# peterdavidfagan/mujoco_robot_environments

Measured on AMD Instinct MI355X. Metric: env steps/sec (whole node), RearrangementEnv batch=4096 at 1/2/4/8 MI355X, higher is better.
Workload: dtype f32

## Files before the change

### mujoco_robot_environments_amd/csrc/mre_kernels.hip

```cpp
#include <hip/hip_runtime.h>

#include "mre_dev.h"
#include "mre_math.h"
#include "mre_collide.h"

namespace mre {
using ModelP = MRE_MODEL_PTR(DevModel);
#if defined(MRE_PHASE_STAMPS) && MRE_PHASE_STAMPS >= 4
__shared__ unsigned long long dbg_acc[4];
#endif

struct OscSm {
  float J[6][7], M[7][7], MiJt[7][6], Li[6][6], Lam[6][6], V[6][6], Jbar[7][6];
  float ep[3], eo[3], F[6], LF[6], tn[7], Jbt[6], xd[6], w[6];
};

struct alignas(8) Blk {
  uint16_t row0;
  uint8_t type, nrows;
  uint8_t rslot;
  uint8_t pa, pb;
  uint8_t primary : 4;
  uint8_t bslot : 4;
};
// ... 18 lines not shown
#endif
  float cdof[NRV][6];
  union {
    struct { float con_pos[NCON_MAX][3], con_frame[NCON_MAX][9], con_dist[NCON_MAX]; };
#ifdef MRE_NEWTON
    struct { float jar[NEFC_MAX], frc[NEFC_MAX], jv[NEFC_MAX]; };
#else
    struct { float jar[NEFC_MAX], frc[NEFC_MAX], pyr_f[4 * NCON_MAX]; };
#endif
  };
  float com_robot[3];
  float site_xpos[NSITE][3], site_xmat[1][9];
#ifdef MRE_NEWTON
  float qM[NMR];
#else
  float qM[NMR], qLD[NMR], qLDinv[NRV + 1];
#endif
  float prop_mass[NPROP], prop_inertia[NPROP][3], prop_size[NPROP][3];
  union { float scratch[64]; int iscr[64]; };
  float osc_tgt[16];
  int nprops;
  int ncon, nefc, nl, nrrow, npp, overflow, solver_iters;
  int finger_contact;
  uint8_t con_pair[NCON_MAX], con_rslot[NCON_MAX], con_bslot[NCON_MAX], con_b1[NCON_MAX], con_b2[NCON_MAX];
  uint16_t lim_info[NRV + 1];
  union {
    float JpA[3 * NCON_MAX][6];
    struct {
      float cinert[NB][10], crb[NRB][10], gP[NRB - GRIP_BODY0][6], gC[NRB - GRIP_BODY0][6];
      double gpose[NRB - GRIP_BODY0][7];
    };
  };
  float JpB[3 * NPP_MAX][6];
  union {
    float Jr[NRROW_MAX][NRV];
    struct {
      float cdof_dot[NV][6], cvel[NB][6], cfrc[NB][6];
      alignas(8) double gI[NRB - GRIP_BODY0][10];
      double gS[NRB - GRIP_BODY0][6];
    };
  };
#ifdef MRE_NEWTON
  float efc_R[NEFC_MAX], efc_aref[NEFC_MAX];
  float frc_r[NRROW_MAX];
  float con_fric[NCON_MAX];
  float hc[NCON_MAX][6];
  float Md[NRV][MD_LD];
  alignas(8) float W[NV * (NV + 1) / 2];
  uint8_t rstate[NEFC_MAX];
  uint8_t clist[NPROP][NCON_MAX];
  uint8_t ccount[NPROP], cpl_robot, cpl_cubes;
  alignas(8) uint16_t jdesc[NEFC_MAX][4];
  float zrow[24];
#else
  float Br[NRROW_MAX][NRV];
  alignas(16) float blkrec[MAXBLK][16];
  Blk blk[MAXBLK];
  uint8_t sched[MAXBLK][8];
#endif
  uint16_t hdr[NEFC_MAX];

  int nblk, nsched;
};

#if defined(MRE_LARGE_CAPS)
static_assert(sizeof(Sm) <= 27136, "large-capacity Sm must fit 6 workgroups per CU");
#else
static_assert(sizeof(Sm) <= 20480, "compact Sm must fit 8 workgroups per CU");
#endif

#ifdef MRE_NEWTON
MRE_DEV float* mh_store(Sm& s) { return &s.JpA[0][0]; }
static_assert(sizeof(((Sm*)0)->JpA) >= sizeof(float) * NMR, "M - h dF/dv fits the head of the constraint block");
#else
MRE_DEV float* mh_store(Sm& s) { return s.qLD; }
#endif

struct BodyRegs {
  float anchor[3], axis[3], xipos[3], ximat[9];
};

MRE_DEV double robot_q(const Sm& s, int d) { return (double)s.qpos[d] + (double)s.qlo[d]; }
MRE_DEV double robot_v(const Sm& s, int d) { return (double)s.qvel[d] + (double)s.qlo[QFINE / 2 + d]; }

MRE_DEV bool prop_is_active(const Sm& s, int propid) { return propid < 0 || propid < s.nprops; }

struct BodyK {
  float quat[4], pos[3], mass, jnt_pos[3], qpos0, jnt_axis[3], ipos[3], iquat[4], inertia[3];
  int qposadr, propid, dofadr, parent;
};
MRE_DEV BodyK load_body(ModelP M, int b) {
  const auto* R = &M->body_rec[b];
  BodyK B;
#pragma unroll
  for (int k = 0; k < 4; k++) { B.quat[k] = R->quat[k]; B.iquat[k] = R->iquat[k]; }
#pragma unroll
  for (int k = 0; k < 3; k++) { B.pos[k] = R->pos[k]; B.jnt_pos[k] = R->jnt_pos[k]; B.jnt_axis[k] = R->jnt_axis[k];
                                B.ipos[k] = R->ipos[k]; B.inertia[k] = R->inertia[k]; }
  B.mass = R->mass; B.qpos0 = R->qpos0; B.qposadr = R->qposadr; B.propid = R->propid; B.dofadr = R->dofadr;
  B.parent = R->parent;
  return B;
}

MRE_DEV bool body_is_active(ModelP M, const Sm& s, int b) {
  int p = M->body_propid[b];
  return p < 0 || p < s.nprops;
}

MRE_DEV void sincos_poly_d(double x, double& sn, double& cs) {
  const double z = x * x;
  double ps = -1.0 / 1307674368000.0;
  ps = ps * z + 1.0 / 6227020800.0;
  ps = ps * z - 1.0 / 39916800.0;
  ps = ps * z + 1.0 / 362880.0;
  ps = ps * z - 1.0 / 5040.0;
  ps = ps * z + 1.0 / 120.0;
  ps = ps * z - 1.0 / 6.0;
  sn = x + x * (z * ps);
  double pc = 1.0 / 20922789888000.0;
  pc = pc * z - 1.0 / 87178291200.0;
  pc = pc * z + 1.0 / 479001600.0;
// ... 1163 lines not shown
  ModelP M = (ModelP)a.M;

  const bool save = a.sv_qpos != nullptr && step_lo == 0;
  if (l < NQP) {
    const float v = a.qpos[(size_t)env * NQP + l];
    s.qpos[l] = v;
    if (save) a.sv_qpos[(size_t)env * NQP + l] = v;
  }
  if (l < NVP) {
    const float v = a.qvel[(size_t)env * NVP + l], w = a.qacc_ws[(size_t)env * NVP + l];
    s.qvel[l] = v;
    s.qacc[l] = w;
    s.qfrc_con[l] = 0.f;
    if (save) { a.sv_qvel[(size_t)env * NVP + l] = v; a.sv_qacc_ws[(size_t)env * NVP + l] = w; }
  }
  if (l < QFINE) {
    const float v = a.qfine != nullptr ? a.qfine[(size_t)env * QFINE_ROW + l] : 0.f;
    s.qlo[l] = v;
    if (save && a.qfine != nullptr) a.sv_qfine[(size_t)env * QFINE_ROW + l] = v;
  }
  if (save && a.qfine != nullptr && l < QFINE_ROW - QFINE)
    a.sv_qfine[(size_t)env * QFINE_ROW + QFINE + l] = a.qfine[(size_t)env * QFINE_ROW + QFINE + l];
  float cube_lo_keep = 0.f;
  if (QUEUE && !Q_LARGE && a.qfine != nullptr && l < QFINE_ROW - QFINE) cube_lo_keep = a.qfine[(size_t)env * QFINE_ROW + QFINE + l];
  if (l < NU) {
    const float v = a.ctrl[(size_t)env * NU + l];
    s.ctrl[l] = v;
    if (save) a.sv_ctrl[(size_t)env * NU + l] = v;
  }
  if (save && l == 0) {
    if (a.nstep != nullptr) a.sv_nstep[env] = a.nstep[env];
    a.sv_status[env] = a.status[env];
    a.sv_converged[env] = a.converged != nullptr ? a.converged[env] : (uint8_t)0;
  }
  if (l == 0) { s.nprops = a.nprops[env]; s.overflow = 0; s.ncon = 0; s.nefc = 0; s.solver_iters = 0; }
#ifdef MRE_NEWTON
  if (l < 24) s.zrow[l] = 0.f;
#endif
  if (l < NPROP * 3) {
    const float sz = a.prop_size[(size_t)env * NPROP * 3 + l];
    s.prop_size[l / 3][l % 3] = sz;
  }
  MRE_SYNC();
  if (l < NPROP) {
    const float m = M->body_mass[NRB + l];
    const float* z = s.prop_size[l];
    s.prop_mass[l] = m;
    s.prop_inertia[l][0] = m / 3.f * (z[1] * z[1] + z[2] * z[2]);
    s.prop_inertia[l][1] = m / 3.f * (z[0] * z[0] + z[2] * z[2]);
    s.prop_inertia[l][2] = m / 3.f * (z[0] * z[0] + z[1] * z[1]);
  }
  MRE_SYNC();

#if defined(MRE_PHASE_STAMPS) && MRE_PHASE_STAMPS >= 4
  if (l < 4) dbg_acc[l] = 0ull;
#endif
#ifdef MRE_PHASE_STAMPS
  unsigned long long stamp_acc[4] = {0, 0, 0, 0};
  unsigned long long stamp_t = __builtin_amdgcn_s_memtime();
#endif
  bool arm_converged = ((a.flags & F_CONV_CONTINUE) != 0 || (QUEUE && qtick > 0)) && a.converged != nullptr && a.converged[env] != 0;
  float grip_cmd = 0.f;
  const OscConfig* oscp = a.osc + (size_t)env * a.osc_stride;
  int hw_ncon = 0, hw_nefc = 0, hw_nrrow = 0, hw_npp = 0;
  const unsigned long long launch_t0 = __builtin_amdgcn_s_memtime();
  if (a.mode == CTRL_OSC) {
    if (l < 16) s.osc_tgt[l] = a.osc_target[(size_t)env * 16 + l];
    grip_cmd = a.grip_closed[env] ? M->act_ctrlrange[NU - 1][1] : M->act_ctrlrange[NU - 1][0];
    MRE_SYNC();
  }
  int steps_done = 0;
  bool settled = false;
  for (int step = step_lo; step < step_hi; ++step) {
    MRE_STAMP(7);
    position_stage(M, s, l);
    MRE_STAMP(12);
    MRE_STAMP(13);
    gripper_local(M, s, l);
    if ((a.flags & F_NO_CONSTRAINTS) == 0) connect_rows_local(M, s, l);
    MRE_STAMP(14);
    crb_mass_matrix(M, s, l);
    MRE_SYNC();
#ifndef MRE_NEWTON
    factor_robot_regs(s.qM, s.qLD, s.qLDinv);
#endif
    MRE_STAMP(15);
    MRE_STAMP(0);

    velocity_stage(M, s, l);
    MRE_SYNC();
    finger_bias(M, s, l);
    MRE_STAMP(1);
    const bool constrained = (a.flags & F_NO_CONSTRAINTS) == 0;
    if (constrained) {

      collide(M, s, l, false, (a.flags & F_CLIP_ALWAYS) != 0);
      MRE_STAMP(2);
      assemble_constraints(M, s, l);
#ifdef MRE_NEWTON
      nw_build_lists(s, l, a.flags);
#else
      solve_robot_rows(s, l);
      assemble_blocks(M, s, l);
#endif
      MRE_STAMP(3);
      hw_ncon = max(hw_ncon, s.ncon); hw_nefc = max(hw_nefc, s.nefc);
// ... 614 lines not shown
```

### mujoco_robot_environments_amd/csrc/mre_newton.h

```cpp
#pragma once

namespace mre {

constexpr int NW_QUAD = 0, NW_SAT = 1, NW_CONE = 4;
constexpr unsigned NW_CPL_ALL_TILES = 0x80u;
constexpr int NW_LS_MAX = 20;
constexpr float NW_LS_TOL = 0.01f;
#ifndef NW_LS_REL_VALUE
#define NW_LS_REL_VALUE 1e-5f
#endif
constexpr float NW_LS_REL = NW_LS_REL_VALUE;

MRE_DEV float rdlane(float v, int lane) {
  return __builtin_bit_cast(float, __builtin_amdgcn_readlane(__builtin_bit_cast(int, v), lane));
}
MRE_DEV int uni(int v) { return __builtin_amdgcn_readfirstlane(v); }
MRE_DEV float unif(float v) {
  return __builtin_bit_cast(float, __builtin_amdgcn_readfirstlane(__builtin_bit_cast(int, v)));
}

MRE_DEV float nw_Jl(const Sm& s, int i, int h, int l, int lp, int lk) {
  const int rs = h & 0xFF, pa = (h >> 8) & 0xF, pb = (h >> 12) & 0xF;
  float j = 0.f;
  if (l < NRV) {
// ... 71 lines not shown
  }
  return o;
}

template <bool FULL, bool PYR>
MRE_DEV float nw_update(Sm& s, int l, int nscalar, int ncon, float mu_scale, const float* jar) {
  constexpr bool pyr = PYR;
  float cost = 0.f;
  if (l < nscalar) {
    const float D = 1.0f / s.efc_R[l], j = jar[l];
    const bool act = l < 7 || j < 0.f;
    if (FULL) {
      const float f = act ? -D * j : 0.f;
      s.frc[l] = f; s.frc_r[l] = f;
      s.rstate[l] = act ? NW_QUAD : NW_SAT;
    }
    cost = act ? 0.5f * D * j * j : 0.f;
  }
  if (l < ncon) {
    const int i = nscalar + 3 * l;
    const float D0 = 1.0f / s.efc_R[i], D1 = 1.0f / s.efc_R[i + 1], D2 = 1.0f / s.efc_R[i + 2];
    const float fr = s.con_fric[l];
    float hc[6];
    const NwContact o = pyr ? nw_pyramid<FULL>(jar[i], jar[i + 1], jar[i + 2], D0, fr, hc)
                            : nw_contact<FULL>(jar[i], jar[i + 1], jar[i + 2], D0, D1, D2, fr, fr * mu_scale, hc);
    cost += o.cost;
    if (FULL) {
      s.frc[i] = o.f0; s.frc[i + 1] = o.f1; s.frc[i + 2] = o.f2;
      const int rs = s.con_rslot[l];
      if (rs != HDR_NONE) { s.frc_r[rs] = o.f0; s.frc_r[rs + 1] = o.f1; s.frc_r[rs + 2] = o.f2; }
      s.rstate[i] = s.rstate[i + 1] = s.rstate[i + 2] = (uint8_t)o.st;
      if (o.st == NW_CONE) {
#pragma unroll
        for (int k = 0; k < 6; k++) s.hc[l][k] = hc[k];
      }
    }
  }
  return wave_sum(cost);
}

struct NwMasks { unsigned long long sc, cq, cc; };
MRE_DEV bool operator==(const NwMasks& a, const NwMasks& b) { return a.sc == b.sc && a.cq == b.cq && a.cc == b.cc; }
MRE_DEV NwMasks nw_masks(const Sm& s, int l, int nscalar, int ncon) {
  NwMasks m;
  const int st_s = l < nscalar ? s.rstate[l] : NW_SAT;
  const int st_c = l < ncon ? s.rstate[nscalar + 3 * l] : NW_SAT;
  m.sc = __ballot(st_s == NW_QUAD);
  m.cq = __ballot(st_c == NW_QUAD);
  m.cc = __ballot(st_c == NW_CONE);
  return m;
}

MRE_DEV float nw_JTf(const Sm& s, int l, int lp, int lk, int nscalar) {
  float acc = 0.f;
  if (l < NRV) {
    const int n = s.nrrow;
    for (int rs = 0; rs < n; rs++) acc = fmaf(s.Jr[rs][l], s.frc_r[rs], acc);
  } else if (l < NV && lp < s.nprops) {
    const int n = s.ccount[lp];
    for (int t = 0; t < n; t++) {
      const int e = s.clist[lp][t], c = e & 0x7F;
      const float* J = (e & 0x80) ? s.JpB[3 * s.con_bslot[c]] : s.JpA[3 * c];
      const float* f = &s.frc[nscalar + 3 * c];
      acc = fmaf(J[lk], f[0], acc);
      acc = fmaf(J[6 + lk], f[1], acc);
      acc = fmaf(J[12 + lk], f[2], acc);
    }
  }
  return acc;
}

MRE_DEV void nw_rank1(float (&hh)[NV], float t, float J, bool has_r, int pa, int pb) {
  if (has_r) {
#pragma unroll
    for (int c = 0; c < NRV; c++) hh[c] = fmaf(t, rdlane(J, c), hh[c]);
  }
#pragma unroll
  for (int p = 0; p < NPROP; p++) {
    if (pa == p || pb == p) {
#pragma unroll
      for (int k = 0; k < 6; k++) hh[NRV + 6 * p + k] = fmaf(t, rdlane(J, NRV + 6 * p + k), hh[NRV + 6 * p + k]);
    }
  }
}

template <int HI, int LO>
MRE_DEV void nw_elim_update(float (&hh)[NV], float u) {
  constexpr int n = HI - LO + 1;
  if constexpr (n > 0) {
#pragma unroll
    for (int g0 = 0; g0 < n; g0 += 8) {
      float t[8];
#pragma unroll
      for (int q = 0; q < 8; q++)
        if (g0 + q < n) t[q] = rdlane(u, HI - g0 - q);
      __builtin_amdgcn_sched_barrier(0);
#pragma unroll
      for (int q = 0; q < 8; q++)
        if (g0 + q < n) hh[HI - g0 - q] = fmaf(-u, t[q], hh[HI - g0 - q]);
      __builtin_amdgcn_sched_barrier(0);
    }
  }
}

template <int K>
MRE_DEV void nw_elim_col(float (&hh)[NV], float& g, float& y, float& dinv, int l, unsigned nbm) {
// ... 11 lines not shown
  if constexpr (blk > 0) {
    if constexpr (blk > 3) { if (nbm & (1u << 3)) nw_elim_update<NRV + 17, NRV + 12>(hh, u); }
    if constexpr (blk > 2) { if (nbm & (1u << 2)) nw_elim_update<NRV + 11, NRV + 6>(hh, u); }
    if constexpr (blk > 1) { if (nbm & (1u << 1)) nw_elim_update<NRV + 5, NRV>(hh, u); }
    if (nbm & 1u) nw_elim_update<NRV - 1, 0>(hh, u);
  }
}
template <int K, int KEND>
MRE_DEV void nw_elim_range(float (&hh)[NV], float& g, float& y, float& dinv, int l, unsigned nbm) {
  nw_elim_col<K>(hh, g, y, dinv, l, nbm);
  if constexpr (K > KEND) nw_elim_range<K - 1, KEND>(hh, g, y, dinv, l, nbm);
}

struct NwPoint { float alpha, cost, d1, d2; };

MRE_PHASE_FN void nw_build_lists(Sm& s, int l, unsigned flags) {
  const int kept = s.ncon;
  const bool on = l < kept;
  const int cb1 = on ? s.con_b1[l] : 0, cb2 = on ? s.con_b2[l] : 0;
  int pa = -1, pb = -1;
  if (cb1 >= NRB) pa = cb1 - NRB;
  if (cb2 >= NRB) { if (pa < 0) pa = cb2 - NRB; else pb = cb2 - NRB; }
  const unsigned long long lt = (1ull << l) - 1ull;
  const bool rob = on && pa >= 0 && s.con_rslot[on ? l : 0] != HDR_NONE;
  unsigned cr = 0u, cc = 0u;
#pragma unroll
  for (int p = 0; p < NPROP; p++) {
    const bool mine = on && (pa == p || pb == p);
    const unsigned long long m = __ballot(mine);
    if (mine) s.clist[p][__popcll(m & lt)] = (uint8_t)(pb == p ? (l | 0x80) : l);
    if (l == 0) s.ccount[p] = (uint8_t)__popcll(m);
    if (__ballot(rob && pa == p) != 0ull) cr |= 1u << p;
  }
  const int pairbit = (on && pb >= 0) ? cube_pair_bit(pa, pb) : -1;
#pragma unroll
  for (int b = 0; b < 6; b++)
    if (__ballot(pairbit == b) != 0ull) cc |= 1u << b;
  if ((flags & F_NW_ALL_TILES) != 0u) cr |= NW_CPL_ALL_TILES;
  if (l == 0) { s.cpl_robot = (uint8_t)cr; s.cpl_cubes = (uint8_t)cc; }
  const int nscalar = 7 + s.nl;
  const unsigned zoff = (unsigned)offsetof(Sm, zrow);
  for (int i = l; i < s.nefc; i += 64) {
    const int h = s.hdr[i], ra = (h >> 8) & 0xF, rb = (h >> 12) & 0xF;
    const int crow = i - nscalar;
    const unsigned offA = crow >= 0 ? (unsigned)offsetof(Sm, JpA) + 24u * (unsigned)crow : zoff;
    const unsigned offB = (crow >= 0 && rb != 0xF)
                              ? (unsigned)offsetof(Sm, JpB) + 24u * (unsigned)(3 * s.con_bslot[crow / 3] + crow % 3) : zoff;
#pragma unroll
    for (int cb = 0; cb < NPROP; cb++) s.jdesc[i][cb] = (uint16_t)(ra == cb ? offA : (rb == cb ? offB : zoff));
  }
  MRE_SYNC();
}

struct NwLane {
  int lp, lk;
  bool lact;
  float mdiag;
  float mu_scale;
  float scale;
};
MRE_DEV NwLane nw_lane(ModelP M, const Sm& s, int l) {
  NwLane c;
  c.lp = (l >= NRV && l < NV) ? (l - NRV) / 6 : -1;
  c.lk = (l >= NRV && l < NV) ? (l - NRV) % 6 : 0;
  c.lact = l < NRV || (c.lp >= 0 && c.lp < s.nprops);
  c.mdiag = c.lp >= 0 ? (c.lk < 3 ? s.prop_mass[c.lp] : s.prop_inertia[c.lp][c.lk - 3]) : 0.f;
  c.mu_scale = __builtin_amdgcn_rsqf(fmaxf(M->opt_rec.impratio, kMinVal));
  float msum = M->opt_rec.M0_diag_robot_sum;
  for (int p = 0; p < s.nprops; p++)
    msum += 3.f * s.prop_mass[p] + s.prop_inertia[p][0] + s.prop_inertia[p][1] + s.prop_inertia[p][2];
  c.scale = 1.0f / msum;
  return c;
}

template <bool PYR>
MRE_DEV float nw_update_gradient(Sm& s, int l, const NwLane& c, int nscalar, int ncon) {
  const float sc = nw_update<true, PYR>(s, l, nscalar, ncon, c.mu_scale, s.jar);
  MRE_SYNC();
  const float qc = nw_JTf(s, l, c.lp, c.lk, nscalar);
  const bool on = l < NV && c.lact;
  const float fs = on ? s.qfrc_smooth[l] : 0.f, as = on ? s.qacc_smooth[l] : 0.f;
  const float qa = on ? s.qacc[l] : 0.f, Ma = on ? s.nw_Ma[l] : 0.f;
  if (l < NVP) {
    s.qfrc_con[l] = on ? qc : 0.f;
    s.nw_grad[l] = on ? Ma - fs - qc : 0.f;
  }
  const float cost = sc + wave_sum(0.5f * (Ma - fs) * (qa - as));
  MRE_SYNC();
  return cost;
}

template <bool PYR>
MRE_DEV float nw_setup_impl(ModelP M, Sm& s, int l) {
  MRE_DBG_T0();
  const NwLane c = nw_lane(M, s, l);
  const int nefc = s.nefc, ncon = s.ncon, nscalar = 7 + s.nl;
  for (int e = l; e < NRV * MD_LD; e += 64) (&s.Md[0][0])[e] = 0.f;
  MRE_SYNC();
  for (int e = l; e < NMR; e += 64) {
    const int i = M->M_i[e], j = M->M_j[e];
    const float v = s.qM[e];
    s.Md[i][j] = v; s.Md[j][i] = v;
  }
  MRE_SYNC();
  MRE_DBG_STAMP(10, 0);
  const bool on = l < NV && c.lact;
  const float fs = on ? s.qfrc_smooth[l] : 0.f, as = on ? s.qacc_smooth[l] : 0.f;
  float qa = on ? s.qacc[l] : 0.f;
  float Ma = on ? nw_mulM(s, l, c.mdiag, s.qacc) : 0.f;
  for (int i = l; i < nefc; i += 64) {
    const float aref = s.efc_aref[i];
    float d1, d2;
    row_dot2(s, i, s.qacc, s.qacc_smooth, d1, d2);
    s.jar[i] = d1 - aref;
    s.jv[i] = d2 - aref;
  }
  MRE_SYNC();
  MRE_DBG_STAMP(10, 1);
  const float gauss = wave_sum(0.5f * (Ma - fs) * (qa - as));
  const float cost_ws = gauss + nw_update<false, PYR>(s, l, nscalar, ncon, c.mu_scale, s.jar);
  const float cost_sm = nw_update<false, PYR>(s, l, nscalar, ncon, c.mu_scale, s.jv);
  const bool smooth_wins = cost_ws > cost_sm || !(cost_ws == cost_ws);
#if defined(MRE_PHASE_STAMPS) && MRE_PHASE_STAMPS == 11
  if (threadIdx.x == 0) { dbg_acc[0] += 1ull << 4; dbg_acc[1] += (unsigned long long)smooth_wins << 4; }
#endif
  if (smooth_wins) {
    qa = as; Ma = fs;
    for (int i = l; i < nefc; i += 64) s.jar[i] = s.jv[i];
  }
  if (l < NVP) { s.qacc[l] = qa; s.nw_Ma[l] = Ma; }
  MRE_SYNC();
  MRE_DBG_STAMP(10, 2);
  const float cost = nw_update_gradient<PYR>(s, l, c, nscalar, ncon);
  MRE_DBG_STAMP(10, 3);
  return cost;
}
MRE_PHASE_FN float nw_setup(ModelP M, Sm& s, int l) { return nw_setup_impl<false>(M, s, l); }
MRE_PHASE_FN float nw_setup_pyramidal(ModelP M, Sm& s, int l) { return nw_setup_impl<true>(M, s, l); }

MRE_PHASE_FN void nw_direction(ModelP M, Sm& s, int l) {
  MRE_DBG_T0();
  const NwLane c = nw_lane(M, s, l);
  const int nefc = s.nefc, nscalar = 7 + s.nl, nprops = s.nprops;
  const int lp = c.lp, lk = c.lk;
  bool t10, t20, t21;
  {
    const unsigned cr = (unsigned)uni((int)s.cpl_robot), cq = (unsigned)uni((int)s.cpl_cubes);
    constexpr unsigned across = (1u << cube_pair_bit(0, 2)) | (1u << cube_pair_bit(0, 3)) | (1u << cube_pair_bit(1, 2)) |
                                (1u << cube_pair_bit(1, 3));
    const bool all_tiles = (cr & NW_CPL_ALL_TILES) != 0u;
    t10 = all_tiles || (cr & 0x3u) != 0u;
    t20 = all_tiles || (cr & 0xCu) != 0u;
    t21 = all_tiles || (cq & across) != 0u;
  }
#if defined(MRE_PHASE_STAMPS) && MRE_PHASE_STAMPS == 9
  if (threadIdx.x == 0) {
    dbg_acc[0] += 1ull << 4; dbg_acc[1] += (unsigned long long)!t10 << 4;
    dbg_acc[2] += (unsigned long long)!t20 << 4; dbg_acc[3] += (unsigned long long)!t21 << 4;
  }
#endif
  float hh[NV];
#pragma unroll
  for (int k = 0; k < NV; k++) {
    float v = 0.f;
    if (k < NRV) { if (l < NRV) v = s.Md[l][k]; }
    else if (l == k) v = c.lact ? c.mdiag : 1.0f;
    hh[k] = v;
  }
  MRE_DBG_STAMP(4, 0);
#if defined(MRE_PHASE_STAMPS) && MRE_PHASE_STAMPS == 5
  {
    int nc_ = 0, nq_ = 0;
    for (int r0 = 0; r0 < nefc; r0 += 64) {
      const int st_ = r0 + l < nefc ? (int)s.rstate[r0 + l] : NW_SAT;
      nc_ += __popcll(__ballot(st_ == NW_CONE)); nq_ += __popcll(__ballot(st_ == NW_QUAD));
    }
    if (threadIdx.x == 0) { dbg_acc[2] += (unsigned long long)nc_ << 4; dbg_acc[3] += (unsigned long long)nq_ << 4; }
  }
#endif
  typedef float v4f __attribute__((ext_vector_type(4)));
  v4f c00 = {0.f, 0.f, 0.f, 0.f}, c10 = c00, c11 = c00, c20 = c00, c21 = c00, c22 = c00;
  {
    const int g = l >> 4, m16 = l & 15;
    const char* const sb = reinterpret_cast<const char*>(&s);
    const unsigned zoff = (unsigned)offsetof(Sm, zrow), jr0 = (unsigned)offsetof(Sm, Jr);
    const unsigned sh = m16 < 12 ? 16u * (unsigned)(m16 / 6) : 0u;
    const unsigned lo = 4u * (unsigned)(m16 % 6), lr = 4u * (unsigned)m16;
    auto ldw = [&](unsigned off) { return *reinterpret_cast<const float*>(sb + off); };
    auto meta = [&](int r0, int& ii, int& st, int& h, float& R, uint2& d) {
      const int i = r0 + g;
      ii = i < nefc ? i : 0;
      st = i < nefc ? (int)s.rstate[ii] : NW_SAT;
      h = s.hdr[ii];
      R = s.efc_R[ii];
      d = *reinterpret_cast<const uint2*>(&s.jdesc[ii][0]);
// ... 123 lines not shown
  unsigned adj[5];
  {
    const unsigned cr = s.cpl_robot, cq = s.cpl_cubes;
    adj[0] = 0u;
#pragma unroll
    for (int p = 0; p < NPROP; p++) {
      unsigned a = (cr >> p) & 1u;
#pragma unroll
      for (int q = 0; q < NPROP; q++)
        if (q != p && ((cq >> cube_pair_bit(p, q)) & 1u)) a |= 1u << (1 + q);
      adj[1 + p] = a;
    }
#pragma unroll
    for (int a = 4; a >= 1; a--) {
      const unsigned nb = adj[a] & ((1u << a) - 1u);
#pragma unroll
      for (int b = 1; b < 4; b++)
        if (b < a && ((nb >> b) & 1u)) adj[b] |= nb & ~(1u << b);
    }
#pragma unroll
    for (int a = 1; a < 5; a++) adj[a] = (unsigned)uni((int)adj[a]);
  }
  float g = l < NVP ? s.nw_grad[l] : 0.f, y = 0.f, dinv = 1.0f;
  if (nprops > 3) nw_elim_range<NRV + 23, NRV + 18>(hh, g, y, dinv, l, adj[4] & 0xFu);
  if (nprops > 2) nw_elim_range<NRV + 17, NRV + 12>(hh, g, y, dinv, l, adj[3] & 0x7u);
  if (nprops > 1) nw_elim_range<NRV + 11, NRV + 6>(hh, g, y, dinv, l, adj[2] & 0x3u);
  if (nprops > 0) nw_elim_range<NRV + 5, NRV>(hh, g, y, dinv, l, adj[1] & 0x1u);
  nw_elim_range<NRV - 1, 0>(hh, g, y, dinv, l, 0u);
  MRE_DBG_STAMP(4, 3);
#pragma unroll
  for (int k = 0; k < NV; k++)
    if (l <= k) s.W[k * (k + 1) / 2 + l] = hh[k];
  MRE_SYNC();
  {
    const int base = l < NV ? l * (l + 1) / 2 : 0;
    const int nva = NRV + 6 * nprops;
#pragma unroll
    for (int j = 0; j < NV - 1; j++) hh[j] = (j < l && l < nva) ? s.W[base + j] : 0.f;
#pragma unroll
    for (int j = 0; j < NV - 1; j++) {
      const float xj = rdlane(y * dinv, j);
      y = fmaf(-hh[j], xj, y);
    }
  }
  const float x = (l < NV && c.lact) ? y * dinv : 0.f;
  if (l < NVP) s.nw_search[l] = -x;
  const float dec = wave_sum((l < NVP ? s.nw_grad[l] : 0.f) * x);
  if (l == 0) s.scratch[2] = dec;
  MRE_SYNC();
  MRE_DBG_STAMP(4, 3);
}

MRE_PHASE_FN void nw_direction_reuse(ModelP M, Sm& s, int l) {
  const NwLane c = nw_lane(M, s, l);
  const int nva = NRV + 6 * s.nprops;
  const bool on = l < NV && c.lact;
  const float gin = on ? s.nw_grad[l] : 0.f;
  float g = gin;
  const float dinv = on ? 1.0f / s.W[l * (l + 1) / 2 + l] : 1.0f;
  float y = 0.f;
  for (int k = nva - 1; k >= 0; k--) {
    const float yk = rdlane(g * dinv, k);
    const float w = (l < k) ? s.W[k * (k + 1) / 2 + l] : 0.f;
    g = fmaf(-w, yk, g);
    y = (l == k) ? yk : y;
  }
  const int base = l < NV ? l * (l + 1) / 2 : 0;
  for (int j = 0; j < nva; j++) {
    const float cw = (j < l && l < NV) ? s.W[base + j] : 0.f;
    const float xj = rdlane(y * dinv, j);
    y = fmaf(-cw, xj, y);
  }
  const float x = on ? y * dinv : 0.f;
  if (l < NVP) s.nw_search[l] = -x;
  const float dec = wave_sum(gin * x);
  if (l == 0) s.scratch[2] = dec;
  MRE_SYNC();
}

template <bool PYR>
MRE_DEV float nw_search_move_impl(ModelP M, Sm& s, int l) {
  MRE_DBG_T0();
  const NwLane c = nw_lane(M, s, l);
  const int nefc = s.nefc, ncon = s.ncon, nscalar = 7 + s.nl;
  const float tol = M->opt_rec.tolerance, mu_scale = c.mu_scale;
  const bool on = l < NV && c.lact;
  const float fs = on ? s.qfrc_smooth[l] : 0.f, as = on ? s.qacc_smooth[l] : 0.f;
  float qa = on ? s.qacc[l] : 0.f, Ma = on ? s.nw_Ma[l] : 0.f;
  const float sv = on ? s.nw_search[l] : 0.f;
  const float Mv = on ? nw_mulM(s, l, c.mdiag, s.nw_search) : 0.f;
  for (int i = l; i < nefc; i += 64) s.jv[i] = row_dot(s, i, s.nw_search);
  MRE_SYNC();
  MRE_DBG_STAMP(7, 0);
  const float snorm = sqrtf(wave_sum(sv * sv));
  float alpha = 0.f;
#if defined(MRE_PHASE_STAMPS) && MRE_PHASE_STAMPS == 7
  int dbg_nev = 0;
#endif
  if (snorm >= kMinVal) {
    const float gtol_abs = tol * NW_LS_TOL * snorm / c.scale;
    float g0 = 0.5f * (Ma - fs) * (qa - as), g1 = sv * (Ma - fs), g2 = 0.5f * sv * Mv;
    wave_sum3(g0, g1, g2);
    float sq0 = 0.f, sq1 = 0.f, sq2 = 0.f, sj = 0.f, svv = 0.f;
    const bool s_on = l < nscalar, s_eq = l < 7;
    if (s_on) {
      const float D = 1.0f / s.efc_R[l];
      sj = s.jar[l]; svv = s.jv[l];
      sq0 = 0.5f * D * sj * sj; sq1 = D * sj * svv; sq2 = 0.5f * D * svv * svv;
    }
    float cq0 = 0.f, cq1 = 0.f, cq2 = 0.f, U0 = 0.f, V0 = 0.f, UU = 0.f, UV = 0.f, VV = 0.f, Dm = 0.f, mu = 0.f;
    const bool c_on = l < ncon;
    constexpr bool pyr = PYR;
    float pe0 = 0.f, pe1 = 0.f, pe2 = 0.f, pe3 = 0.f, pv0 = 0.f, pv1 = 0.f, pv2 = 0.f, pv3 = 0.f, pD = 0.f;
    if (c_on && pyr) {
      const int i = nscalar + 3 * l;
      const float fr = s.con_fric[l];
      const float j0 = s.jar[i], j1 = fr * s.jar[i + 1], j2 = fr * s.jar[i + 2];
      const float v0 = s.jv[i], v1 = fr * s.jv[i + 1], v2 = fr * s.jv[i + 2];
      pe0 = j0 + j1; pe1 = j0 - j1; pe2 = j0 + j2; pe3 = j0 - j2;
      pv0 = v0 + v1; pv1 = v0 - v1; pv2 = v0 + v2; pv3 = v0 - v2;
      pD = 1.0f / s.efc_R[i];
    }
    if (c_on && !pyr) {
      const int i = nscalar + 3 * l;
      const float fr = s.con_fric[l];
      mu = fr * mu_scale;
#pragma unroll
      for (int r = 0; r < 3; r++) {
        const float D = 1.0f / s.efc_R[i + r], j = s.jar[i + r], v = s.jv[i + r];
        cq0 += 0.5f * D * j * j; cq1 += D * j * v; cq2 += 0.5f * D * v * v;
      }
      const float U1 = s.jar[i + 1] * fr, U2 = s.jar[i + 2] * fr, V1 = s.jv[i + 1] * fr, V2 = s.jv[i + 2] * fr;
      U0 = s.jar[i] * mu; V0 = s.jv[i] * mu;
      UU = U1 * U1 + U2 * U2; UV = U1 * V1 + U2 * V2; VV = V1 * V1 + V2 * V2;
      Dm = (1.0f / s.efc_R[i]) / fmaxf(mu * mu * (1.f + mu * mu), kMinVal);
    }
#if defined(MRE_PHASE_STAMPS) && MRE_PHASE_STAMPS == 7
#define NW_DBG_EVAL() dbg_nev++
#else
#define NW_DBG_EVAL() do {} while (0)
#endif
    auto eval = [&](float a) {
      NW_DBG_EVAL();
      float q0 = 0.f, q1 = 0.f, q2 = 0.f, ec = 0.f, e1 = 0.f, e2 = 0.f;
      if (s_on && (s_eq || sj + a * svv < 0.f)) { q0 = sq0; q1 = sq1; q2 = sq2; }
      if (c_on && pyr) {
        const float x0 = fminf(pe0 + a * pv0, 0.f), x1 = fminf(pe1 + a * pv1, 0.f);
        const float x2 = fminf(pe2 + a * pv2, 0.f), x3 = fminf(pe3 + a * pv3, 0.f);
        ec = 0.5f * pD * ((x0 * x0 + x1 * x1) + (x2 * x2 + x3 * x3));
        e1 = pD * ((x0 * pv0 + x1 * pv1) + (x2 * pv2 + x3 * pv3));
        e2 = pD * (((x0 < 0.f ? pv0 * pv0 : 0.f) + (x1 < 0.f ? pv1 * pv1 : 0.f)) +
                   ((x2 < 0.f ? pv2 * pv2 : 0.f) + (x3 < 0.f ? pv3 * pv3 : 0.f)));
      }
// ... 15 lines not shown
            ec = 0.5f * Dm * NT * NT;
            e1 = Dm * NT * w;
            e2 = Dm * (w * w - NT * mu * T2);
          }
        }
        if (quad) { q0 += cq0; q1 += cq1; q2 += cq2; }
      }
      NwPoint p;
      p.alpha = a;
      float s0 = ec + q0 + a * (q1 + a * q2), s1 = e1 + q1 + 2.f * a * q2, s2 = e2 + 2.f * q2;
      wave_sum3(s0, s1, s2);
      p.cost = s0 + g0 + a * (g1 + a * g2);
      p.d1 = s1 + g1 + 2.f * a * g2;
      p.d2 = s2 + 2.f * g2;
      return p;
    };
    const NwPoint p0 = eval(0.f);
    if (p0.d2 >= kMinVal) {
      const float gtol = fmaxf(gtol_abs, NW_LS_REL * fabsf(p0.d1));
      NwPoint p1 = eval(-p0.d1 / p0.d2);
      if (!(p1.cost <= p0.cost)) p1 = p0;
      if (fabsf(p1.d1) < gtol) {
        alpha = p1.alpha;
      } else {
        NwPoint lo = p0, hi = p0;
        bool have_lo = p0.d1 < 0.f, have_hi = !have_lo;
        bool found = false;
        for (int it = 0; it < NW_LS_MAX; it++) {
          if (p1.d1 < 0.f) { if (!have_lo || p1.alpha > lo.alpha) { lo = p1; have_lo = true; } }
          else { if (!have_hi || p1.alpha < hi.alpha) { hi = p1; have_hi = true; } }
          float a = p1.alpha - p1.d1 / p1.d2;
          if (have_lo && have_hi && !(a > lo.alpha && a < hi.alpha)) a = 0.5f * (lo.alpha + hi.alpha);
          if (fabsf(a - p1.alpha) <= 2e-7f * fabsf(p1.alpha)) break;
          p1 = eval(a);
          if (fabsf(p1.d1) < gtol) { found = true; break; }
        }
        if (found) alpha = p1.alpha;
        else if (have_lo && have_hi) alpha = lo.cost < hi.cost ? lo.alpha : hi.alpha;
        else alpha = p1.cost < p0.cost ? p1.alpha : 0.f;
      }
    }
  }
  if (l == 0) { s.scratch[0] = alpha; s.scratch[1] = 0.f; }
  MRE_DBG_STAMP(7, 1);
#if defined(MRE_PHASE_STAMPS) && MRE_PHASE_STAMPS == 7
  if (threadIdx.x == 0) dbg_acc[3] += (unsigned long long)dbg_nev << 4;
#endif
  if (alpha == 0.f) { MRE_SYNC(); return 0.f; }
  qa = fmaf(alpha, sv, qa);
  Ma = fmaf(alpha, Mv, Ma);
  if (l < NVP) { s.qacc[l] = qa; s.nw_Ma[l] = Ma; }
  for (int i = l; i < nefc; i += 64) s.jar[i] = fmaf(alpha, s.jv[i], s.jar[i]);
  MRE_SYNC();
  const float cost = nw_update_gradient<PYR>(s, l, c, nscalar, ncon);
  const float gr = l < NVP ? s.nw_grad[l] : 0.f;
  const float gn = sqrtf(wave_sum(gr * gr));
  if (l == 0) s.scratch[1] = gn;
  MRE_SYNC();
  MRE_DBG_STAMP(7, 2);
  return cost;
}
MRE_PHASE_FN float nw_search_move(ModelP M, Sm& s, int l) { return nw_search_move_impl<false>(M, s, l); }
MRE_PHASE_FN float nw_search_move_pyramidal(ModelP M, Sm& s, int l) { return nw_search_move_impl<true>(M, s, l); }

#ifdef MRE_PHASE_STAMPS
#define NW_STAMP(k)                                                          \
  do {                                                                       \
    const unsigned long long now_ = __builtin_amdgcn_s_memtime();            \
    if ((8 + (k)) / 4 == MRE_PHASE_STAMPS) stamp_acc[(k) % 4] += now_ - stamp_t; \
    stamp_t = now_;                                                          \
  } while (0)
MRE_DEV void newton_solve(ModelP M, Sm& s, int l, unsigned long long* stamp_acc, unsigned long long& stamp_t) {
#else
#define NW_STAMP(k) do {} while (0)
MRE_DEV void newton_solve(ModelP M, Sm& s, int l) {
#endif
  const float tol = M->opt_rec.tolerance;
  const int max_iter = M->opt_rec.iterations;
  const int nscalar = 7 + s.nl, ncon = s.ncon;
  float msum = M->opt_rec.M0_diag_robot_sum;
  for (int p = 0; p < s.nprops; p++)
    msum += 3.f * s.prop_mass[p] + s.prop_inertia[p][0] + s.prop_inertia[p][1] + s.prop_inertia[p][2];
  const float scale = 1.0f / msum;
  const bool pyr = M->opt_rec.cone == 0;
  if (pyr) nw_setup_pyramidal(M, s, l);
  else nw_setup(M, s, l);
  NW_STAMP(0);
#ifndef NW_TOL_FACTOR
#define NW_TOL_FACTOR 1.0f
#endif
  const float tol_eff = NW_TOL_FACTOR * tol;
  NwMasks mf = {0ull, 0ull, 0ull}, mprev = {~0ull, ~0ull, ~0ull};
  bool have_factor = false, force_full = false;
  float prev_dec = 3.0e38f;
  int iter = 0, nfull = 0, stalls = 0;
  while (iter < max_iter) {
    const NwMasks mk = nw_masks(s, l, nscalar, ncon);
    const bool reuse = have_factor && !force_full && mk == mf && mk.cc == 0ull;
    if (reuse) {
      nw_direction_reuse(M, s, l);
      NW_STAMP(2);
    } else {
      nw_direction(M, s, l);
      mf = mk; have_factor = true; nfull++;
      NW_STAMP(1);
    }
    const float dec = s.scratch[2];
    if (!(dec == dec)) break;
    if (0.5f * scale * dec < tol_eff) break;
    if (mk == mprev && dec > 0.1f * prev_dec) {
      if (reuse) { force_full = true; continue; }
      if (0.5f * scale * dec < 100.f * tol_eff && ++stalls >= 2) break;
    }
    prev_dec = dec; mprev = mk; force_full = false;
    if (pyr) nw_search_move_pyramidal(M, s, l);
    else nw_search_move(M, s, l);
    NW_STAMP(3);
    const float alpha = s.scratch[0];
    if (alpha == 0.f) {
      if (reuse) { force_full = true; continue; }
      break;
    }
    iter++;
    if (!reuse && mk.cc == 0ull && fabsf(alpha - 1.0f) < 1e-4f && nw_masks(s, l, nscalar, ncon) == mk) break;
  }
  if (l < NVP && !(l < NV)) s.qacc[l] = 0.f;
  if (l == 0) s.solver_iters = iter | (nfull << 8);
  MRE_SYNC();
}

MRE_DEV double rdlane_d(double v, int lane) {
  const long long b = __builtin_bit_cast(long long, v);
  const int lo = __builtin_amdgcn_readlane((int)(b & 0xFFFFFFFFll), lane);
  const int hi = __builtin_amdgcn_readlane((int)(b >> 32), lane);
  return __builtin_bit_cast(double, ((long long)hi << 32) | (long long)(unsigned)lo);
}
MRE_DEV double rcp_d(double x) {
  double r = __builtin_amdgcn_rcp(x);
  r = fma(fma(-x, r, 1.0), r, r);
  r = fma(fma(-x, r, 1.0), r, r);
  return r;
}
MRE_PHASE_FN bool nw_robot_polish(ModelP M, Sm& s, int l) {
  static_assert(offsetof(Sm, W) % 8 == 0 && offsetof(Sm, nw_Mv) % 8 == 0, "fp64 views of W / nw_Mv");
  constexpr int MAXROW = 7 + NRV;
  constexpr int NW_POLISH_CON = 32;
  static_assert(sizeof(((Sm*)0)->W) >= 8 * (2 * MAXROW + 10 * NW_POLISH_CON), "exchange area");
  static_assert(sizeof(((Sm*)0)->nw_Mv) >= 8 * NRV, "fp64 accelerations out");
  double* const frow = reinterpret_cast<double*>(&s.W[0]);
  double* const drow = frow + MAXROW;
  double* const fcon = drow + MAXROW;
  double* const a64 = reinterpret_cast<double*>(&s.nw_Mv[0]);
  const int nscalar = 7 + s.nl, ncon = s.ncon;
  constexpr int F0 = GRIP_BODY0 - 1;
  int nrc = 0;
  bool full = false;
  {
    const int rs = l < ncon ? (int)s.con_rslot[l] : HDR_NONE;
    const bool mine = rs != HDR_NONE;
    const unsigned long long m = __ballot(mine);
    nrc = __popcll(m);
    if (nrc > NW_POLISH_CON) return false;
    const int cb1 = mine ? (int)s.con_b1[l] : 0, cb2 = mine ? (int)s.con_b2[l] : 0;
    full = __ballot(mine && ((cb1 >= 1 && cb1 < GRIP_BODY0) || (cb2 >= 1 && cb2 < GRIP_BODY0))) != 0ull;
#ifdef MRE_POLISH_FULL
    full = true;
#endif
    if (mine) {
      const int k = __popcll(m & ((1ull << l) - 1ull));
      const int i = nscalar + 3 * l, h = s.hdr[i];
      const int pa = (h >> 8) & 0xF, pb = (h >> 12) & 0xF;
      double j[3], D[3];
#pragma unroll
      for (int r = 0; r < 3; r++) {
        double acc = -(double)s.efc_aref[i + r];
#pragma unroll
        for (int c = 0; c < NRV; c++) acc += (double)s.Jr[rs + r][c] * (double)s.qacc[c];
        if (pa < NPROP) { const float* ja = jpA(s, i + r); for (int c = 0; c < 6; c++) acc += (double)ja[c] * (double)s.qacc[NRV + 6 * pa + c]; }
        if (pb < NPROP) { const float* jb = jpB(s, i + r); for (int c = 0; c < 6; c++) acc += (double)jb[c] * (double)s.qacc[NRV + 6 * pb + c]; }
        j[r] = acc;
        D[r] = rcp_d((double)s.efc_R[i + r]);
      }
      const double fr = (double)s.con_fric[l], mu = fr * sqrt((double)s.efc_R[i + 1] / (double)s.efc_R[i]);
      const double U1 = j[1] * fr, U2 = j[2] * fr, Nn = j[0] * mu, T = sqrt(U1 * U1 + U2 * U2);
      double* o = fcon + 10 * k;
#pragma unroll
      for (int t = 0; t < 9; t++) o[t] = 0.0;
      o[9] = (double)rs;
      if (M->opt_rec.cone == 0) {
        const double e[4] = {j[0] + fr * j[1], j[0] - fr * j[1], j[0] + fr * j[2], j[0] - fr * j[2]};
        double a[4], n[4];
#pragma unroll
        for (int t = 0; t < 4; t++) { a[t] = e[t] < 0.0 ? e[t] : 0.0; n[t] = e[t] < 0.0 ? 1.0 : 0.0; }
        o[0] = -D[0] * (a[0] + a[1] + a[2] + a[3]);
        o[1] = -D[0] * fr * (a[0] - a[1]);
        o[2] = -D[0] * fr * (a[2] - a[3]);
        o[3] = D[0] * (n[0] + n[1] + n[2] + n[3]);
        o[4] = D[0] * fr * (n[0] - n[1]);
        o[5] = D[0] * fr * (n[2] - n[3]);
        o[6] = D[0] * fr * fr * (n[0] + n[1]);
        o[8] = D[0] * fr * fr * (n[2] + n[3]);
      } else if (Nn >= mu * T || (T <= 0.0 && Nn >= 0.0)) {
      } else if (mu * Nn + T <= 0.0 || (T <= 0.0 && Nn < 0.0)) {
        o[0] = -D[0] * j[0]; o[1] = -D[1] * j[1]; o[2] = -D[2] * j[2];
        o[3] = D[0]; o[6] = D[1]; o[8] = D[2];
      } else {
        const double Dm = D[0] / fmax(mu * mu * (1.0 + mu * mu), 1e-15), NT = Nn - mu * T, iT = 1.0 / T;
        o[0] = -Dm * NT * mu;
        o[1] = -o[0] * iT * U1 * fr;
        o[2] = -o[0] * iT * U2 * fr;
        const double a = mu * Nn * iT * iT * iT, dgn = mu * mu - mu * Nn * iT;
        o[3] = Dm * mu * mu;
        o[4] = Dm * mu * fr * (-mu * U1 * iT);
        o[5] = Dm * mu * fr * (-mu * U2 * iT);
        o[6] = Dm * fr * fr * (a * U1 * U1 + dgn);
        o[7] = Dm * fr * fr * (a * U1 * U2);
        o[8] = Dm * fr * fr * (a * U2 * U2 + dgn);
      }
    }
  }
  if (l < nscalar) {
    double jar = -(double)s.efc_aref[l];
#pragma unroll
    for (int j = 0; j < NRV; j++) jar += (double)s.Jr[l][j] * (double)s.qacc[j];
    const bool act = l < 7 || s.rstate[l] == NW_QUAD;
    const double D = act ? rcp_d((double)s.efc_R[l]) : 0.0;
    frow[l] = -D * jar;
    drow[l] = D;
  }
  MRE_SYNC();
  const int d = l < NRV ? l : 0;
  const bool row = l < NRV && (full || l >= F0);
  double hrow[NRV], g = 0.0;
#pragma unroll
  for (int j = 0; j < NRV; j++) hrow[j] = row ? (double)s.Md[d][j] : 0.0;
  if (row) {
    g = -(double)s.qfrc_smooth[d];
#pragma unroll
    for (int j = 0; j < NRV; j++) g += (double)s.Md[d][j] * (double)s.qacc[j];
    for (int r = 0; r < nscalar; r++) {
      const double jd = (double)s.Jr[r][d];
      g -= jd * frow[r];
// ... 75 lines not shown
```

Measured before the change: 25.19 million.

## Cache Newton solver constants in shared memory and batch J^T f loads

Computes the solver's model-derived constants (impratio-based mu scale, mass-sum scale, tolerance, iteration count, cone type) once per work item and stores them in shared memory. Phases then read them as wave-uniform values instead of reloading model fields and recomputing the mass sum in every call. The J^T f reduction is rewritten to process four rows or contact-list entries per iteration, issuing all loads before the FMAs to expose more memory parallelism. When the all-tiles coupling flag is set it falls back to the original per-call path; the batched loop adds tail handling and register pressure.

```diff
diff --git a/mujoco_robot_environments_amd/csrc/mre_kernels.hip b/mujoco_robot_environments_amd/csrc/mre_kernels.hip
--- a/mujoco_robot_environments_amd/csrc/mre_kernels.hip
+++ b/mujoco_robot_environments_amd/csrc/mre_kernels.hip
@@ -94,6 +94,8 @@
   uint8_t ccount[NPROP], cpl_robot, cpl_cubes;
   alignas(8) uint16_t jdesc[NEFC_MAX][4];
   float zrow[24];
+  float nw_scale, nw_mu_scale, nw_tol;
+  int nw_iter, nw_cone;
 #else
   float Br[NRROW_MAX][NRV];
   alignas(16) float blkrec[MAXBLK][16];
@@ -109,6 +111,11 @@
 static_assert(sizeof(Sm) <= 27136, "large-capacity Sm must fit 6 workgroups per CU");
 #else
 static_assert(sizeof(Sm) <= 20480, "compact Sm must fit 8 workgroups per CU");
+#endif
+
+#ifdef MRE_NEWTON
+static_assert(offsetof(Sm, nw_scale) >= offsetof(Sm, JpA) + sizeof(float) * 64 * COLL_BUF && offsetof(Sm, zrow) < offsetof(Sm, nw_scale),
+              "written once per item: no phase of the step may run over them");
 #endif
 
 #ifdef MRE_NEWTON
@@ -1378,6 +1385,9 @@
   }
   MRE_SYNC();
 
+#ifdef MRE_NEWTON
+  nw_item_constants(M, s, l);
+#endif
 #if defined(MRE_PHASE_STAMPS) && MRE_PHASE_STAMPS >= 4
   if (l < 4) dbg_acc[l] = 0ull;
 #endif
diff --git a/mujoco_robot_environments_amd/csrc/mre_newton.h b/mujoco_robot_environments_amd/csrc/mre_newton.h
--- a/mujoco_robot_environments_amd/csrc/mre_newton.h
+++ b/mujoco_robot_environments_amd/csrc/mre_newton.h
@@ -147,6 +147,61 @@
 }
 
 MRE_DEV float nw_JTf(const Sm& s, int l, int lp, int lk, int nscalar) {
+  static_assert(offsetof(Sm, clist) % 4 == 0 && NCON_MAX % 4 == 0, "four list entries in one word");
+  float acc = 0.f;
+  if (l < NRV) {
+    const int n = uni(s.nrrow);
+    const float* Jl = &s.Jr[0][l];
+    int rs = 0;
+    for (; rs + 4 <= n; rs += 4) {
+      const float j0 = Jl[NRV * rs], j1 = Jl[NRV * (rs + 1)], j2 = Jl[NRV * (rs + 2)], j3 = Jl[NRV * (rs + 3)];
+      const float f0 = s.frc_r[rs], f1 = s.frc_r[rs + 1], f2 = s.frc_r[rs + 2], f3 = s.frc_r[rs + 3];
+      acc = fmaf(j0, f0, acc); acc = fmaf(j1, f1, acc); acc = fmaf(j2, f2, acc); acc = fmaf(j3, f3, acc);
+    }
+    if (rs < n) {
+      const int r1 = rs + 1 < n ? rs + 1 : rs, r2 = rs + 2 < n ? rs + 2 : rs;
+      const float j0 = Jl[NRV * rs], j1 = Jl[NRV * r1], j2 = Jl[NRV * r2];
+      const float f0 = s.frc_r[rs], f1 = s.frc_r[r1], f2 = s.frc_r[r2];
+      acc = fmaf(j0, f0, acc);
+      if (rs + 1 < n) acc = fmaf(j1, f1, acc);
+      if (rs + 2 < n) acc = fmaf(j2, f2, acc);
+    }
+  } else if (l < NV && lp < s.nprops) {
+    const int n = s.ccount[lp];
+    for (int t0 = 0; t0 < n; t0 += 4) {
+      const unsigned w = *reinterpret_cast<const unsigned*>(&s.clist[lp][t0]);
+      int e[4], b[4];
+#pragma unroll
+      for (int q = 0; q < 4; q++) e[q] = t0 + q < n ? (int)((w >> (8 * q)) & 0xFFu) : (int)(w & 0xFFu);
+#pragma unroll
+      for (int q = 0; q < 4; q++) b[q] = 0;
+      if (((e[0] | e[1] | e[2] | e[3]) & 0x80) != 0) {
+#pragma unroll
+        for (int q = 0; q < 4; q++) b[q] = (e[q] & 0x80) ? (int)s.con_bslot[e[q] & 0x7F] : 0;
+      }
+      float J0[4], J1[4], J2[4], f0[4], f1[4], f2[4];
+#pragma unroll
+      for (int q = 0; q < 4; q++) {
+        const int c = e[q] & 0x7F;
+        const float* J = ((e[q] & 0x80) ? s.JpB[3 * b[q]] : s.JpA[3 * c]) + lk;
+        const float* f = &s.frc[nscalar + 3 * c];
+        J0[q] = J[0]; J1[q] = J[6]; J2[q] = J[12];
+        f0[q] = f[0]; f1[q] = f[1]; f2[q] = f[2];
+      }
+#pragma unroll
+      for (int q = 0; q < 4; q++) {
+        if (t0 + q < n) {
+          acc = fmaf(J0[q], f0[q], acc);
+          acc = fmaf(J1[q], f1[q], acc);
+          acc = fmaf(J2[q], f2[q], acc);
+        }
+      }
+    }
+  }
+  return acc;
+}
+
+MRE_DEV float nw_JTf_serial(const Sm& s, int l, int lp, int lk, int nscalar) {
   float acc = 0.f;
   if (l < NRV) {
     const int n = s.nrrow;
@@ -264,32 +319,82 @@
   MRE_SYNC();
 }
 
+struct NwOpt {
+  float mu_scale;
+  float scale;
+  float tol;
+  int iterations, cone;
+  bool generic;
+};
+MRE_DEV NwOpt nw_opt_model(ModelP M, const Sm& s) {
+  NwOpt o;
+  o.mu_scale = __builtin_amdgcn_rsqf(fmaxf(M->opt_rec.impratio, kMinVal));
+  float msum = M->opt_rec.M0_diag_robot_sum;
+  for (int p = 0; p < s.nprops; p++)
+    msum += 3.f * s.prop_mass[p] + s.prop_inertia[p][0] + s.prop_inertia[p][1] + s.prop_inertia[p][2];
+  o.scale = 1.0f / msum;
+  o.tol = M->opt_rec.tolerance;
+  o.iterations = M->opt_rec.iterations;
+  o.cone = M->opt_rec.cone;
+  o.generic = true;
+  return o;
+}
+MRE_DEV void nw_item_constants(ModelP M, Sm& s, int l) {
+  const NwOpt o = nw_opt_model(M, s);
+  if (l == 0) { s.nw_scale = o.scale; s.nw_mu_scale = o.mu_scale; s.nw_tol = o.tol; s.nw_iter = o.iterations; s.nw_cone = o.cone; }
+  MRE_SYNC();
+}
+struct NwOptWords { float mu_scale, scale, tol; int iterations, cone, cpl; };
+MRE_DEV NwOptWords nw_opt_read(const Sm& s) {
+  NwOptWords w;
+  w.mu_scale = s.nw_mu_scale; w.scale = s.nw_scale; w.tol = s.nw_tol;
+  w.iterations = s.nw_iter; w.cone = s.nw_cone; w.cpl = s.cpl_robot;
+  return w;
+}
+MRE_DEV NwOpt nw_opt(ModelP M, const Sm& s, const NwOptWords& w) {
+  if ((uni(w.cpl) & (int)NW_CPL_ALL_TILES) != 0) return nw_opt_model(M, s);
+  NwOpt o;
+  o.mu_scale = unif(w.mu_scale); o.scale = unif(w.scale); o.tol = unif(w.tol);
+  o.iterations = uni(w.iterations); o.cone = uni(w.cone);
+  o.generic = false;
+  return o;
+}
+MRE_DEV NwOpt nw_opt(ModelP M, const Sm& s) { return nw_opt(M, s, nw_opt_read(s)); }
+
 struct NwLane {
   int lp, lk;
   bool lact;
   float mdiag;
-  float mu_scale;
-  float scale;
 };
-MRE_DEV NwLane nw_lane(ModelP M, const Sm& s, int l) {
+MRE_DEV NwLane nw_lane(const Sm& s, int l) {
   NwLane c;
   c.lp = (l >= NRV && l < NV) ? (l - NRV) / 6 : -1;
   c.lk = (l >= NRV && l < NV) ? (l - NRV) % 6 : 0;
   c.lact = l < NRV || (c.lp >= 0 && c.lp < s.nprops);
   c.mdiag = c.lp >= 0 ? (c.lk < 3 ? s.prop_mass[c.lp] : s.prop_inertia[c.lp][c.lk - 3]) : 0.f;
-  c.mu_scale = __builtin_amdgcn_rsqf(fmaxf(M->opt_rec.impratio, kMinVal));
-  float msum = M->opt_rec.M0_diag_robot_sum;
-  for (int p = 0; p < s.nprops; p++)
-    msum += 3.f * s.prop_mass[p] + s.prop_inertia[p][0] + s.prop_inertia[p][1] + s.prop_inertia[p][2];
-  c.scale = 1.0f / msum;
   return c;
 }
 
-template <bool PYR>
-MRE_DEV float nw_update_gradient(Sm& s, int l, const NwLane& c, int nscalar, int ncon) {
-  const float sc = nw_update<true, PYR>(s, l, nscalar, ncon, c.mu_scale, s.jar);
-  MRE_SYNC();
-  const float qc = nw_JTf(s, l, c.lp, c.lk, nscalar);
+#if defined(MRE_PHASE_STAMPS) && MRE_PHASE_STAMPS >= 4
+#define NW_DBG_CLOCK_ARG , unsigned long long& dbg_t_
+#define NW_DBG_CLOCK , dbg_t_
+#define NW_UG_STAMP(SET, K) do { if (MRE_PHASE_STAMPS == (SET)) MRE_DBG_STAMP(SET, K); } while (0)
+#else
+#define NW_DBG_CLOCK_ARG
+#define NW_DBG_CLOCK
+#define NW_UG_STAMP(SET, K) do {} while (0)
+#endif
+template <bool PYR, int SET>
+MRE_DEV float nw_update_gradient(Sm& s, int l, const NwLane& c, const NwOpt& o, int nscalar, int ncon NW_DBG_CLOCK_ARG) {
+  const float sc = nw_update<true, PYR>(s, l, nscalar, ncon, o.mu_scale, s.jar);
+  MRE_SYNC();
+  NW_UG_STAMP(SET, 0);
+#ifdef NW_JTF_ONE_BY_ONE
+  const float qc = nw_JTf_serial(s, l, c.lp, c.lk, nscalar);
+#else
+  const float qc = o.generic ? nw_JTf_serial(s, l, c.lp, c.lk, nscalar) : nw_JTf(s, l, c.lp, c.lk, nscalar);
+#endif
+  NW_UG_STAMP(SET, 1);
   const bool on = l < NV && c.lact;
   const float fs = on ? s.qfrc_smooth[l] : 0.f, as = on ? s.qacc_smooth[l] : 0.f;
   const float qa = on ? s.qacc[l] : 0.f, Ma = on ? s.nw_Ma[l] : 0.f;
@@ -299,13 +404,15 @@
   }
   const float cost = sc + wave_sum(0.5f * (Ma - fs) * (qa - as));
   MRE_SYNC();
+  NW_UG_STAMP(SET, 2);
   return cost;
 }
 
 template <bool PYR>
 MRE_DEV float nw_setup_impl(ModelP M, Sm& s, int l) {
   MRE_DBG_T0();
-  const NwLane c = nw_lane(M, s, l);
+  const NwLane c = nw_lane(s, l);
+  const NwOptWords ow = nw_opt_read(s);
   const int nefc = s.nefc, ncon = s.ncon, nscalar = 7 + s.nl;
   for (int e = l; e < NRV * MD_LD; e += 64) (&s.Md[0][0])[e] = 0.f;
   MRE_SYNC();
@@ -328,10 +435,11 @@
     s.jv[i] = d2 - aref;
   }
   MRE_SYNC();
+  const NwOpt o = nw_opt(M, s, ow);
   MRE_DBG_STAMP(10, 1);
   const float gauss = wave_sum(0.5f * (Ma - fs) * (qa - as));
-  const float cost_ws = gauss + nw_update<false, PYR>(s, l, nscalar, ncon, c.mu_scale, s.jar);
-  const float cost_sm = nw_update<false, PYR>(s, l, nscalar, ncon, c.mu_scale, s.jv);
+  const float cost_ws = gauss + nw_update<false, PYR>(s, l, nscalar, ncon, o.mu_scale, s.jar);
+  const float cost_sm = nw_update<false, PYR>(s, l, nscalar, ncon, o.mu_scale, s.jv);
   const bool smooth_wins = cost_ws > cost_sm || !(cost_ws == cost_ws);
 #if defined(MRE_PHASE_STAMPS) && MRE_PHASE_STAMPS == 11
   if (threadIdx.x == 0) { dbg_acc[0] += 1ull << 4; dbg_acc[1] += (unsigned long long)smooth_wins << 4; }
@@ -343,7 +451,7 @@
   if (l < NVP) { s.qacc[l] = qa; s.nw_Ma[l] = Ma; }
   MRE_SYNC();
   MRE_DBG_STAMP(10, 2);
-  const float cost = nw_update_gradient<PYR>(s, l, c, nscalar, ncon);
+  const float cost = nw_update_gradient<PYR, 12>(s, l, c, o, nscalar, ncon NW_DBG_CLOCK);
   MRE_DBG_STAMP(10, 3);
   return cost;
 }
@@ -352,7 +460,7 @@
 
 MRE_PHASE_FN void nw_direction(ModelP M, Sm& s, int l) {
   MRE_DBG_T0();
-  const NwLane c = nw_lane(M, s, l);
+  const NwLane c = nw_lane(s, l);
   const int nefc = s.nefc, nscalar = 7 + s.nl, nprops = s.nprops;
   const int lp = c.lp, lk = c.lk;
   bool t10, t20, t21;
@@ -582,7 +690,7 @@
 }
 
 MRE_PHASE_FN void nw_direction_reuse(ModelP M, Sm& s, int l) {
-  const NwLane c = nw_lane(M, s, l);
+  const NwLane c = nw_lane(s, l);
   const int nva = NRV + 6 * s.nprops;
   const bool on = l < NV && c.lact;
   const float gin = on ? s.nw_grad[l] : 0.f;
@@ -611,9 +719,9 @@
 template <bool PYR>
 MRE_DEV float nw_search_move_impl(ModelP M, Sm& s, int l) {
   MRE_DBG_T0();
-  const NwLane c = nw_lane(M, s, l);
+  const NwLane c = nw_lane(s, l);
+  const NwOptWords ow = nw_opt_read(s);
   const int nefc = s.nefc, ncon = s.ncon, nscalar = 7 + s.nl;
-  const float tol = M->opt_rec.tolerance, mu_scale = c.mu_scale;
   const bool on = l < NV && c.lact;
   const float fs = on ? s.qfrc_smooth[l] : 0.f, as = on ? s.qacc_smooth[l] : 0.f;
   float qa = on ? s.qacc[l] : 0.f, Ma = on ? s.nw_Ma[l] : 0.f;
@@ -621,6 +729,8 @@
   const float Mv = on ? nw_mulM(s, l, c.mdiag, s.nw_search) : 0.f;
   for (int i = l; i < nefc; i += 64) s.jv[i] = row_dot(s, i, s.nw_search);
   MRE_SYNC();
+  const NwOpt o = nw_opt(M, s, ow);
+  const float tol = o.tol, mu_scale = o.mu_scale;
   MRE_DBG_STAMP(7, 0);
   const float snorm = sqrtf(wave_sum(sv * sv));
   float alpha = 0.f;
@@ -628,7 +738,7 @@
   int dbg_nev = 0;
 #endif
   if (snorm >= kMinVal) {
-    const float gtol_abs = tol * NW_LS_TOL * snorm / c.scale;
+    const float gtol_abs = tol * NW_LS_TOL * snorm / o.scale;
     float g0 = 0.5f * (Ma - fs) * (qa - as), g1 = sv * (Ma - fs), g2 = 0.5f * sv * Mv;
     wave_sum3(g0, g1, g2);
     float sq0 = 0.f, sq1 = 0.f, sq2 = 0.f, sj = 0.f, svv = 0.f;
@@ -750,7 +860,8 @@
   if (l < NVP) { s.qacc[l] = qa; s.nw_Ma[l] = Ma; }
   for (int i = l; i < nefc; i += 64) s.jar[i] = fmaf(alpha, s.jv[i], s.jar[i]);
   MRE_SYNC();
-  const float cost = nw_update_gradient<PYR>(s, l, c, nscalar, ncon);
+  NW_UG_STAMP(13, 3);
+  const float cost = nw_update_gradient<PYR, 13>(s, l, c, o, nscalar, ncon NW_DBG_CLOCK);
   const float gr = l < NVP ? s.nw_grad[l] : 0.f;
   const float gn = sqrtf(wave_sum(gr * gr));
   if (l == 0) s.scratch[1] = gn;
@@ -773,14 +884,11 @@
 #define NW_STAMP(k) do {} while (0)
 MRE_DEV void newton_solve(ModelP M, Sm& s, int l) {
 #endif
-  const float tol = M->opt_rec.tolerance;
-  const int max_iter = M->opt_rec.iterations;
+  const NwOpt o = nw_opt(M, s);
+  const float tol = o.tol, scale = o.scale;
+  const int max_iter = o.iterations;
   const int nscalar = 7 + s.nl, ncon = s.ncon;
-  float msum = M->opt_rec.M0_diag_robot_sum;
-  for (int p = 0; p < s.nprops; p++)
-    msum += 3.f * s.prop_mass[p] + s.prop_inertia[p][0] + s.prop_inertia[p][1] + s.prop_inertia[p][2];
-  const float scale = 1.0f / msum;
-  const bool pyr = M->opt_rec.cone == 0;
+  const bool pyr = o.cone == 0;
   if (pyr) nw_setup_pyramidal(M, s, l);
   else nw_setup(M, s, l);
   NW_STAMP(0);
@@ -850,6 +958,7 @@
   double* const fcon = drow + MAXROW;
   double* const a64 = reinterpret_cast<double*>(&s.nw_Mv[0]);
   const int nscalar = 7 + s.nl, ncon = s.ncon;
+  const int cone = nw_opt(M, s).cone;
   constexpr int F0 = GRIP_BODY0 - 1;
   int nrc = 0;
   bool full = false;
@@ -885,7 +994,7 @@
 #pragma unroll
       for (int t = 0; t < 9; t++) o[t] = 0.0;
       o[9] = (double)rs;
-      if (M->opt_rec.cone == 0) {
+      if (cone == 0) {
         const double e[4] = {j[0] + fr * j[1], j[0] - fr * j[1], j[0] + fr * j[2], j[0] - fr * j[2]};
         double a[4], n[4];
 #pragma unroll
```

After: 25.35 million, median of 6. Within noise of the previous version (+0.6%).
